# Edresson/VoiceSplit

Hardware: AMD Instinct MI355X
Metric: utterances/sec (3 s clips, B=64/GPU) fwd+bwd, channels-last bf16 activations / tape, bf16 MFMA, fp32 accumulate / statistics / master weights (higher is better)
Workload: dtype bf16 (conv activations and tape stored as bf16; bf16 MFMA operands in the convs, the LSTM / head contractions and the BPTT, f16 operands in the forward recurrence; fp32 accumulate, BatchNorm statistics, gate arithmetic / cell state, loss head, master weights)

## Files before the change

include/voicesplit_hip.h:

```cpp
#ifndef VOICESPLIT_HIP_H
#define VOICESPLIT_HIP_H

#include <stddef.h>
#include <stdint.h>

#ifdef __cplusplus
extern "C" {
#endif
#if defined(__GNUC__)
#pragma GCC visibility push(default)
#endif

#define VS_ABI_VERSION 10

#define VS_ACT_RELU 0
#define VS_ACT_MISH 1
#define VS_ACT_NONE 2
#define VS_ACT_SIGMOID 3

#define VS_MATH_FP32 0
#define VS_MATH_F16X3 1
#define VS_MATH_BF16 2

#define VS_BN_EVAL 0
#define VS_BN_TRAIN 1

typedef struct vs_dims {
  int B;
// ... 140 lines not shown
int vs_nhwc_bn_act_bwd(const void* da, const void* z, void* dz, long long npix, int act, int bn_mode,
                       const float* scale, const float* shift, const float* mean, const float* invstd,
                       float* dgamma, float* dbeta, float* dbias, double* stats, float* coef, void* stream);
int vs_nhwc_bn_act_bwd_first(const void* da, const void* z, const float* x, int B, int T, int F, int act, int bn_mode,
                             const float* scale, const float* shift, const float* mean, const float* invstd,
                             float* dgamma, float* dbeta, float* dbias, float* dw, double* stats, float* coef, double* acc, void* stream);
int vs_nhwc_conv_last_bwd_blocks(void);
int vs_nhwc_conv_last_bwd(const float* dz8, const float* w, const void* a7, void* din, float* partials, float* dw,
                          int B, int T, int F, void* stream);
int vs_nhwc_conv_dy(const void* dz, const void* packed, void* dy, const void* z, int act,
                    const float* bn_scale, const float* bn_shift, const float* bn_mean, const float* bn_invstd, double* bn_stats,
                    int B, int T, int F, int KT, int KF, int dil, void* stream);
int vs_nhwc_conv_last_bwd_dy(const float* dz8, const float* w, const void* a7, void* dy, float* partials, float* dw,
                             const void* z7, int act, const float* bn_scale, const float* bn_shift, const float* bn_mean,
                             const float* bn_invstd, double* bn_stats, int B, int T, int F, void* stream);
int vs_nhwc_bn_bwd_from_dy(const void* dy, const void* z, void* dz, long long npix, int bn_mode,
                           const float* scale, const float* mean, const float* invstd,
                           float* dgamma, float* dbeta, float* dbias, double* stats, float* coef, void* stream);
int vs_nhwc_bn_bwd_first_from_dy(const void* dy, const void* z, const float* x, int B, int T, int F, int bn_mode,
                                 const float* scale, const float* mean, const float* invstd,
                                 float* dgamma, float* dbeta, float* dbias, float* dw, double* stats, float* coef, double* acc, void* stream);
int vs_conv_last_fwd(const float* in, const float* w, const float* scale, const float* shift,
                     float* out, int B, int T, int F, int act, void* stream);
int vs_gemm_nt(const float* A, int lda, const float* W, int ldw, float* C, int ldc, int M, int N, int K,
               const float* bias1, const float* bias2, const float* rowbias, int ldrb, int group,
               int a_relu, int act, void* stream);
size_t vs_lstm_packed_floats(int H);
size_t vs_lstm_state_floats(int B, int H);
int vs_lstm_pack(const float* w_hh_fwd, const float* w_hh_bwd, float* packed, int H, void* stream);
int vs_bilstm_recurrent(const float* xg, const float* packed_whh, float* state, float* out,
// ... 149 lines not shown
```

voicesplit_amd/_lib.py:

```python
import ctypes
import os
from ctypes import POINTER, Structure, c_char_p, c_float, c_int, c_longlong, c_size_t, c_void_p

_HERE = os.path.dirname(os.path.abspath(__file__))
LIB_PATH = os.path.join(_HERE, "libvoicesplit_hip.so")

ACT_RELU, ACT_MISH, ACT_NONE, ACT_SIGMOID = 0, 1, 2, 3
BN_EVAL, BN_TRAIN = 0, 1
MATH_FP32, MATH_F16X3, MATH_BF16 = 0, 1, 2
PROF_SLOTS = 29
PROF_NAMES = ("cnn1", "cnn2", "cnn3", "cnn4", "cnn5", "cnn6", "cnn7", "cnn8", "lstm_gemm", "lstm_rec", "head",
              "fwd_bn", "bwd_head", "bwd_lstm_rec", "bwd_lstm_gemm", "bwd_bn",
              "wgrad_cnn2", "wgrad_cnn3", "wgrad_cnn4", "wgrad_cnn5", "wgrad_cnn6", "wgrad_cnn7",
              "dgrad_cnn2", "dgrad_cnn3", "dgrad_cnn4", "dgrad_cnn5", "dgrad_cnn6", "dgrad_cnn7", "bwd_edge")
ABI_VERSION = 10


class VsDims(Structure):
    _fields_ = [(n, c_int) for n in ("B", "T", "F", "E", "H", "FC1", "FC2", "math")]


class VsConvLayer(Structure):
    _fields_ = [(n, c_void_p) for n in ("weight", "bias", "bn_weight", "bn_bias",
                                        "bn_running_mean", "bn_running_var")]


class VsParams(Structure):
    _fields_ = [
        ("conv", VsConvLayer * 8),
        ("w_ih", c_void_p * 2), ("w_hh", c_void_p * 2), ("b_ih", c_void_p * 2), ("b_hh", c_void_p * 2),
# ... 83 lines not shown
    "vs_nhwc_first_stats": (c_int, [_P, _P, _P, ctypes.c_double, _P, _P]),
    "vs_nhwc_first_bwd_scratch_doubles": (c_int, []),
    "vs_nhwc_first_bwd": (c_int, [_P, _P, _P, _P, c_int, c_int, c_int, c_int, c_int, _P, _P, _P, _P, _P, _P, _P, _P, _P, _P]),
    "vs_bn_finalize": (c_int, [_P, c_int, ctypes.c_double, c_int, _P, _P, _P, _P, c_float, c_float, _P, _P, _P, _P, _P]),
    "vs_nhwc_bn_apply": (c_int, [_P, _P, c_longlong, c_int, _P, _P, _P]),
    "vs_nhwc_conv_last": (c_int, [_P, _P, _P, _P, _P, c_int, c_int, c_int, c_int, _P]),
    "vs_nhwc_conv_last_pre": (c_int, [_P, _P, _P, c_int, _P, _P, _P, _P, _P, c_int, c_int, c_int, _P]),
    "vs_nhwc_conv_wgrad_partial_floats": (c_size_t, [c_int, c_int]),
    "vs_nhwc_conv_wgrad": (c_int, [_P, _P, _P, _P, c_int, c_int, c_int, c_int, c_int, c_int, _P]),
    "vs_nhwc_bn_act_bwd": (c_int, [_P, _P, _P, c_longlong, c_int, c_int, _P, _P, _P, _P, _P, _P, _P, _P, _P, _P]),
    "vs_nhwc_bn_act_bwd_first": (c_int, [_P, _P, _P, c_int, c_int, c_int, c_int, c_int, _P, _P, _P, _P, _P, _P, _P, _P, _P, _P, _P, _P]),
    "vs_nhwc_conv_last_bwd_blocks": (c_int, []),
    "vs_nhwc_conv_last_bwd": (c_int, [_P, _P, _P, _P, _P, _P, c_int, c_int, c_int, _P]),
    "vs_nhwc_conv_dy": (c_int, [_P, _P, _P, _P, c_int, _P, _P, _P, _P, _P, c_int, c_int, c_int, c_int, c_int, c_int, _P]),
    "vs_nhwc_conv_last_bwd_dy": (c_int, [_P, _P, _P, _P, _P, _P, _P, c_int, _P, _P, _P, _P, _P, c_int, c_int, c_int, _P]),
    "vs_nhwc_bn_bwd_from_dy": (c_int, [_P, _P, _P, c_longlong, c_int, _P, _P, _P, _P, _P, _P, _P, _P, _P]),
    "vs_nhwc_bn_bwd_first_from_dy": (c_int, [_P, _P, _P, c_int, c_int, c_int, c_int, _P, _P, _P, _P, _P, _P, _P, _P, _P, _P, _P]),
    "vs_conv_last_fwd": (c_int, [_P, _P, _P, _P, _P, c_int, c_int, c_int, c_int, _P]),
    "vs_conv64_packed_f16_floats": (c_size_t, [c_int, c_int]),
    "vs_pow2_scale": (c_int, [_P, c_longlong, _P, _P, _P]),
    "vs_conv64_pack_f16": (c_int, [_P, _P, c_int, c_int, c_int, _P, _P, _P]),
    "vs_conv64_f16x3_fwd": (c_int, [_P, _P, _P, _P, _P, _P, _P, c_int, c_int, c_int, c_int, c_int, c_int, c_int, _P]),
    "vs_gemm_nt": (c_int, [_P, c_int, _P, c_int, _P, c_int, c_int, c_int, c_int, _P, _P, _P, c_int, c_int,
                           c_int, c_int, _P]),
    "vs_lstm_packed_floats": (c_size_t, [c_int]),
    "vs_lstm_state_floats": (c_size_t, [c_int, c_int]),
    "vs_lstm_pack": (c_int, [_P, _P, _P, c_int, _P]),
    "vs_bilstm_recurrent": (c_int, [_P, _P, _P, _P, c_int, c_int, c_int, _P]),
    "vs_lstm_pack_math": (c_int, [_P, _P, _P, c_int, c_int, _P]),
    "vs_bilstm_recurrent_math": (c_int, [_P, _P, _P, _P, _P, _P, c_int, c_int, c_int, c_int, _P]),
# ... 114 lines not shown
```

voicesplit_amd/csrc/capi.hip:

```cpp
#include <stdarg.h>
#include <stdlib.h>
#include <string.h>

#include "../../include/voicesplit_hip.h"
#include "vs_internal.h"

static thread_local char g_err[512] = "";

void vs_set_error(const char* fmt, ...) {
  va_list ap;
  va_start(ap, fmt);
  vsnprintf(g_err, sizeof(g_err), fmt, ap);
  va_end(ap);
}

int g_vs_options[VS_OPT_COUNT] = { 1,  1,  1,  1,  0,  0};
thread_local unsigned* g_vs_turn = nullptr;

namespace {
struct Prof {
  bool on = false;
  int max_calls = 0;
  int calls[VS_PROF_SLOTS] = {0};
  hipEvent_t* ev = nullptr;
// ... 450 lines not shown
  return vs_nhwc_bn_act_bwd_impl(da, z, dz, npix, act, bn_mode == VS_BN_TRAIN, scale, shift, mean, invstd, dgamma, dbeta, dbias,
                                 stats, coef, (hipStream_t)stream);
}

int vs_nhwc_bn_act_bwd_first(const void* da, const void* z, const float* x, int B, int T, int F, int act, int bn_mode,
                             const float* scale, const float* shift, const float* mean, const float* invstd,
                             float* dgamma, float* dbeta, float* dbias, float* dw, double* stats, float* coef, double* acc, void* stream) {
  return vs_nhwc_bn_act_bwd_first_impl(da, z, x, B, T, F, act, bn_mode == VS_BN_TRAIN, scale, shift, mean, invstd, dgamma, dbeta, dbias,
                                       dw, stats, coef, acc, (hipStream_t)stream);
}

int vs_nhwc_conv_last_bwd_blocks(void) { return VS_NHWC_LAST_BWD_BLOCKS; }

int vs_nhwc_conv_last_bwd(const float* dz8, const float* w, const void* a7, void* din, float* partials, float* dw,
                          int B, int T, int F, void* stream) {
  return vs_nhwc_conv_last_bwd_impl(dz8, w, a7, din, partials, dw, B, T, F, nullptr, VS_ACT_NONE, nullptr, nullptr, nullptr, nullptr, nullptr,
                                    (hipStream_t)stream);
}

int vs_nhwc_conv_dy(const void* dz, const void* packed, void* dy, const void* z, int act,
                    const float* bn_scale, const float* bn_shift, const float* bn_mean, const float* bn_invstd, double* bn_stats,
                    int B, int T, int F, int KT, int KF, int dil, void* stream) {
  VS_REQUIRE(dz != dy, "nhwc_conv_dy: in-place is not supported");
  return vs_nhwc_conv_dy_impl(dz, packed, dy, z, act, bn_scale, bn_shift, bn_mean, bn_invstd, bn_stats, B, T, F, KT, KF, dil, (hipStream_t)stream);
}

int vs_nhwc_conv_last_bwd_dy(const float* dz8, const float* w, const void* a7, void* dy, float* partials, float* dw,
                             const void* z7, int act, const float* bn_scale, const float* bn_shift, const float* bn_mean,
                             const float* bn_invstd, double* bn_stats, int B, int T, int F, void* stream) {
  VS_REQUIRE(z7, "nhwc_conv_last_bwd_dy: NULL z7");
  return vs_nhwc_conv_last_bwd_impl(dz8, w, a7, dy, partials, dw, B, T, F, z7, act, bn_scale, bn_shift, bn_mean, bn_invstd, bn_stats,
                                    (hipStream_t)stream);
}

int vs_nhwc_bn_bwd_from_dy(const void* dy, const void* z, void* dz, long long npix, int bn_mode,
                           const float* scale, const float* mean, const float* invstd,
                           float* dgamma, float* dbeta, float* dbias, double* stats, float* coef, void* stream) {
  return vs_nhwc_bn_bwd_from_dy_impl(dy, z, dz, npix, bn_mode == VS_BN_TRAIN, scale, mean, invstd, dgamma, dbeta, dbias, stats, coef,
                                     (hipStream_t)stream);
}

int vs_nhwc_bn_bwd_first_from_dy(const void* dy, const void* z, const float* x, int B, int T, int F, int bn_mode,
                                 const float* scale, const float* mean, const float* invstd,
                                 float* dgamma, float* dbeta, float* dbias, float* dw, double* stats, float* coef, double* acc, void* stream) {
  return vs_nhwc_bn_bwd_first_from_dy_impl(dy, z, x, B, T, F, bn_mode == VS_BN_TRAIN, scale, mean, invstd, dgamma, dbeta, dbias, dw,
                                           stats, coef, acc, (hipStream_t)stream);
}
// ... 393 lines not shown
```

voicesplit_amd/csrc/nhwc_edge.hip:

```cpp
#include "vs_internal.h"

namespace {

typedef unsigned u4v __attribute__((ext_vector_type(4)));
typedef unsigned u2v __attribute__((ext_vector_type(2)));

__device__ __forceinline__ float bf_lo(unsigned u) { return __uint_as_float(u << 16); }
__device__ __forceinline__ float bf_hi(unsigned u) { return __uint_as_float(u & 0xffff0000u); }

template <int NV>
__device__ __forceinline__ void fold_channel_sums(float (&v)[NV][8], double* __restrict__ stats, float* lds ,
                                                  unsigned* turn = nullptr) {
  const int lane = threadIdx.x & 63, wave = threadIdx.x >> 6;
#pragma unroll
  for (int q = 0; q < NV; ++q)
#pragma unroll
    for (int j = 0; j < 8; ++j) {
      float s = v[q][j];
      s += __shfl_xor(s, 8, 64);
      s += __shfl_xor(s, 16, 64);
      s += __shfl_xor(s, 32, 64);
      if (lane < 8) lds[(wave * NV + q) * 64 + lane * 8 + j] = s;
    }
  __syncthreads();
// ... 373 lines not shown
    const vs_f32x2 u = {__builtin_amdgcn_exp2f(e.x), __builtin_amdgcn_exp2f(e.y)};
    const vs_f32x2 n = u * (u + 2.0f);
    const vs_f32x2 dn = n + 2.0f;
    const vs_f32x2 r = {__builtin_amdgcn_rcpf(dn.x), __builtin_amdgcn_rcpf(dn.y)};
    a = y * (n * r);
    d = r * __builtin_elementwise_fma((yc * 4.0f) * r, __builtin_elementwise_fma(u, u, u), n);
  } else if (ACT == VS_ACT_RELU) {
    a = vs_f32x2{fmaxf(y.x, 0.0f), fmaxf(y.y, 0.0f)};
    d = vs_f32x2{y.x > 0.0f ? 1.0f : 0.0f, y.y > 0.0f ? 1.0f : 0.0f};
  } else {
    a = y;
    d = vs_f32x2{1.0f, 1.0f};
  }
}

template <int DYACT, bool RECOMP = false>
__global__ __launch_bounds__(256)
void nhwc_conv_last_bwd_kernel(const float* __restrict__ dz8, const float* __restrict__ w, const u4v* __restrict__ a7,
                               u4v* __restrict__ din, float* __restrict__ part, long long npix, int F, LastBwdBn bn) {
  __shared__ float red[4 * 8 * 64];
  const int piece = threadIdx.x & 7;
  vs_f32x2 wr[8][4], acc[8][4];
  vs_f32x2 sc[4], sh[4], mu[4], is[4], bacc[2][4];
#pragma unroll
  for (int co = 0; co < 8; ++co)
#pragma unroll
    for (int q = 0; q < 4; ++q) {
      wr[co][q] = vs_f32x2{w[co * 64 + piece * 8 + 2 * q], w[co * 64 + piece * 8 + 2 * q + 1]};
      acc[co][q] = vs_f32x2{0.f, 0.f};
    }
  if (DYACT >= 0) {
// ... 28 lines not shown
    if (fn >= F) { fn -= F; ++rown; }
    const long long pn = p + stride;
    if (pn < npix) fetch(pn, rown, fn, nxt);
    vs_f32x2 zf[4], dact[4];
    u4v av = cur.av;
    if (DYACT >= 0) {
#pragma unroll
      for (int q = 0; q < 4; ++q) {
        zf[q] = vs_f32x2{bf_lo(cur.zv[q]), bf_hi(cur.zv[q])};
        vs_f32x2 aq;
        nhwc_act_both2<(DYACT >= 0 ? DYACT : VS_ACT_NONE)>(__builtin_elementwise_fma(zf[q], sc[q], sh[q]), aq, dact[q]);
        if (RECOMP) av[q] = vs_pack_bf16(aq.x, aq.y);
      }
    }
    vs_f32x2 g[4];
#pragma unroll
    for (int q = 0; q < 4; ++q) g[q] = vs_f32x2{0.f, 0.f};
#pragma unroll
    for (int co = 0; co < 8; ++co) {
      const vs_f32x2 dd = {cur.d[co], cur.d[co]};
#pragma unroll
      for (int q = 0; q < 4; ++q) {
        g[q] = __builtin_elementwise_fma(wr[co][q], dd, g[q]);
        acc[co][q] = __builtin_elementwise_fma(dd, vs_f32x2{bf_lo(av[q]), bf_hi(av[q])}, acc[co][q]);
      }
    }
    if (DYACT >= 0) {
#pragma unroll
      for (int q = 0; q < 4; ++q) {
        g[q] *= dact[q];
        bacc[0][q] += g[q];
        bacc[1][q] = __builtin_elementwise_fma(g[q], (zf[q] - mu[q]) * is[q], bacc[1][q]);
      }
    }
    __builtin_nontemporal_store(u4v{vs_pack_bf16(g[0].x, g[0].y), vs_pack_bf16(g[1].x, g[1].y), vs_pack_bf16(g[2].x, g[2].y), vs_pack_bf16(g[3].x, g[3].y)},
                                din + p * 8 + piece);
    cur = nxt;
    f = fn;
    row = rown;
  }
  if (DYACT >= 0) {
    float b8[2][8];
#pragma unroll
    for (int q = 0; q < 4; ++q) {
      b8[0][2 * q] = bacc[0][q].x; b8[0][2 * q + 1] = bacc[0][q].y;
      b8[1][2 * q] = bacc[1][q].x; b8[1][2 * q + 1] = bacc[1][q].y;
    }
    fold_channel_sums<2>(b8, bn.stats, red, bn.turn);
    __syncthreads();
  }
  const int lane = threadIdx.x & 63, wave = threadIdx.x >> 6;
#pragma unroll
  for (int co = 0; co < 8; ++co)
#pragma unroll
    for (int j = 0; j < 8; ++j) {
      float s = (j & 1) ? acc[co][j >> 1].y : acc[co][j >> 1].x;
      s += __shfl_xor(s, 8, 64);
      s += __shfl_xor(s, 16, 64);
      s += __shfl_xor(s, 32, 64);
      if (lane < 8) red[(wave * 8 + co) * 64 + lane * 8 + j] = s;
    }
  __syncthreads();
  for (int i = threadIdx.x; i < 512; i += 256)
    part[(size_t)blockIdx.x * 512 + i] = red[i] + red[512 + i] + red[1024 + i] + red[1536 + i];
}

constexpr int kMomN = 7 + 28;

__global__ __launch_bounds__(256)
void nhwc_first_moments_kernel(const float* __restrict__ x, long long npix, int F, double* __restrict__ mom, unsigned* turn) {
  __shared__ float red[4][kMomN];
  float acc[kMomN];
#pragma unroll
  for (int i = 0; i < kMomN; ++i) acc[i] = 0.f;
  const long long stride = (long long)gridDim.x * 256;
  for (long long p = (long long)blockIdx.x * 256 + threadIdx.x; p < npix; p += stride) {
    const int f = (int)(p % F);
    const float* xr = x + (p - f);
    float xv[7];
// ... 404 lines not shown
  }
  if (int rc = vs_bn_bwd_finalize_impl(stats, VS_BN_STAT_SLOTS, (double)npix, train, 64, scale, mean, invstd, dgamma, dbeta, dbias, coef, stream)) return rc;
  VS_CHECK_HIP(hipMemsetAsync(acc, 0, sizeof(double) * 448, stream));
  const dim3 grid(stream_blocks(32, npix)), block(256);
  if (act == VS_ACT_MISH) hipLaunchKernelGGL(nhwc_bn_bwd_first_kernel<VS_ACT_MISH>, grid, block, 0, stream, g, zz, x, npix, F, scale, shift, coef, acc);
  else if (act == VS_ACT_RELU) hipLaunchKernelGGL(nhwc_bn_bwd_first_kernel<VS_ACT_RELU>, grid, block, 0, stream, g, zz, x, npix, F, scale, shift, coef, acc);
  else hipLaunchKernelGGL(nhwc_bn_bwd_first_kernel<VS_ACT_NONE>, grid, block, 0, stream, g, zz, x, npix, F, scale, shift, coef, acc);
  hipLaunchKernelGGL(nhwc_cvt_f64_f32_kernel, dim3(2), dim3(256), 0, stream, acc, dw, 448);
  VS_LAUNCH_CHECK();
  return 0;
}

int vs_nhwc_conv_last_bwd_impl(const float* dz8, const float* w, const void* a7, void* din, float* part, float* dw,
                               int B, int T, int F, const void* z7, int act, const float* bn_scale, const float* bn_shift,
                               const float* bn_mean, const float* bn_invstd, double* bn_stats, hipStream_t stream) {
  VS_REQUIRE(dz8 && w && din && part && dw, "nhwc conv_last_bwd: NULL argument");
  VS_REQUIRE(a7 || z7, "nhwc conv_last_bwd: a7 may only be NULL in the dy form (it is then recomputed from z7)");
  VS_REQUIRE(!z7 || (bn_scale && bn_shift && bn_mean && bn_invstd && bn_stats), "nhwc conv_last_bwd: the dy form needs the BatchNorm constants and statistics slots");
  const long long npix = (long long)B * T * F;
  long long nb = (npix + 31) / 32;
  if (nb > VS_NHWC_LAST_BWD_BLOCKS) nb = VS_NHWC_LAST_BWD_BLOCKS;
  const LastBwdBn bn{reinterpret_cast<const u4v*>(z7), bn_scale, bn_shift, bn_mean, bn_invstd, bn_stats, z7 ? g_vs_turn : nullptr};
  const dim3 grid((unsigned)nb), block(256);
  const u4v* a = reinterpret_cast<const u4v*>(a7);
  u4v* o = reinterpret_cast<u4v*>(din);
  if (!z7) hipLaunchKernelGGL(nhwc_conv_last_bwd_kernel<-1>, grid, block, 0, stream, dz8, w, a, o, part, npix, F, bn);
  else if (act == VS_ACT_MISH && !a7) hipLaunchKernelGGL((nhwc_conv_last_bwd_kernel<VS_ACT_MISH, true>), grid, block, 0, stream, dz8, w, a, o, part, npix, F, bn);
  else if (act == VS_ACT_RELU && !a7) hipLaunchKernelGGL((nhwc_conv_last_bwd_kernel<VS_ACT_RELU, true>), grid, block, 0, stream, dz8, w, a, o, part, npix, F, bn);
  else if (act == VS_ACT_MISH) hipLaunchKernelGGL(nhwc_conv_last_bwd_kernel<VS_ACT_MISH>, grid, block, 0, stream, dz8, w, a, o, part, npix, F, bn);
  else if (act == VS_ACT_RELU) hipLaunchKernelGGL(nhwc_conv_last_bwd_kernel<VS_ACT_RELU>, grid, block, 0, stream, dz8, w, a, o, part, npix, F, bn);
  else VS_REQUIRE(false, "nhwc conv_last_bwd: dy form for activation %d", act);
  VS_LAUNCH_CHECK();
  return vs_reduce_partials_impl(part, (int)nb, 512, dw, stream);
}

namespace {

typedef _Float16 h8v __attribute__((ext_vector_type(8)));
typedef _Float16 h2v __attribute__((ext_vector_type(2)));

__global__ void nhwc_first_plan_kernel(const unsigned* __restrict__ amax_in, int n_amax, const float* __restrict__ w, const float* __restrict__ scale,
                                       const float* __restrict__ shift, float* __restrict__ out_scale2, int nco, int taps) {
  const int c = threadIdx.x;
  unsigned mb = 0;
  for (int i = c; i < n_amax; i += 64) mb = amax_in[i] > mb ? amax_in[i] : mb;
#pragma unroll
  for (int o = 32; o > 0; o >>= 1) { const unsigned other = __shfl_xor(mb, o, 64); mb = other > mb ? other : mb; }
  float bound = 0.3125f;
// ... 265 lines not shown
```

voicesplit_amd/csrc/train.hip:

```cpp
#include <mutex>
#include <stdlib.h>
#include <string.h>

#include "../../include/voicesplit_hip.h"
#include "vs_internal.h"

int vs_check_dims_impl(const vs_dims* d);

namespace {

constexpr float kBnEps = 1e-5f;
constexpr float kBnMomentum = 0.1f;
struct Spec { int kt, kf, dil; };
constexpr Spec kMid[6] = {{7, 1, 1}, {5, 5, 1}, {5, 5, 2}, {5, 5, 4}, {5, 5, 8}, {5, 5, 16}};
constexpr int kSplitK = 16;

inline size_t align_up(size_t x) { return (x + 255) & ~size_t(255); }
template <typename T>
inline T* at(void* ws, size_t off) { return reinterpret_cast<T*>(static_cast<char*>(ws) + off); }
inline size_t max3(size_t a, size_t b, size_t c) { return a > b ? (a > c ? a : c) : (b > c ? b : c); }

int tape_layout(const vs_dims* d, vs_tape_layout* L) {
  if (int rc = vs_check_dims_impl(d)) return rc;
  memset(L, 0, sizeof(*L));
// ... 562 lines not shown
  auto bn_bwd = [&](int l, const float* da, const float* z, float* dz, int C, long long R, int Lrow) -> int {
    VsProfScope ps(VS_PROF_BWD_BN, stream);
    unsigned* amax = (f16 && l >= 1 && l <= 6) ? vs_amax_slot(cs + VS_SCALE_SLOT_FLOATS * (8 + l)) : nullptr;
    return vs_bn_act_bwd_impl(da, z, dz, C, R, Lrow, conv_act, train, scale + 64 * l, shift + 64 * l, mean + 64 * l,
                              invstd + 64 * l, g->conv[l].bn_weight, g->conv[l].bn_bias, g->conv[l].bias, stats, coef, amax, stream);
  };
  if (int rc = bn_bwd(7, dfeat, at<float>(tape, L.z8), dfeat, 8, (long long)M * 8, F)) return rc;
  if (d->math == VS_MATH_BF16) {
    const long long npix = (long long)B * T * F;
    void* gb[2] = {at<void>(tape, L.grad0), at<void>(tape, L.grad1)};
    int c = 0;
    constexpr int kStatsDoubles = 0;
    {
      VsProfScope ps(VS_PROF_BWD_EDGE, stream);
      VS_CHECK_HIP(hipMemsetAsync(stats, 0, sizeof(double) * VS_BN_STAT_SLOTS * 128, stream));
      if (int rc = vs_nhwc_conv_last_bwd_impl(dfeat, p->conv[7].weight, train ? nullptr : at<void>(tape, L.a[6]), gb[c], at<float>(tape, L.grad1),
                                              g->conv[7].weight, B, T, F, at<void>(tape, L.z[6]), conv_act, scale + 64 * 6, shift + 64 * 6,
                                              mean + 64 * 6, invstd + 64 * 6, stats, stream)) return rc;
    }
    {
      auto from_dy = [&](int l, void* gbuf, hipStream_t s, int beside) -> int {
        VsProfScope ps(VS_PROF_BWD_BN, s);
        return vs_nhwc_bn_bwd_from_dy_impl(gbuf, at<void>(tape, L.z[l]), gbuf, npix, train, scale + 64 * l, mean + 64 * l, invstd + 64 * l,
                                           g->conv[l].bn_weight, g->conv[l].bn_bias, g->conv[l].bias, stats, coef, s, kStatsDoubles, beside);
      };
      auto first_bwd = [&](void* gbuf, hipStream_t s) -> int {
        VsProfScope ps(VS_PROF_BWD_EDGE, s);
        return vs_nhwc_first_bwd_impl(gbuf, x, p->conv[0].weight, p->conv[0].bias, B, T, F, conv_act, train, scale, shift, mean, invstd,
                                      g->conv[0].bn_weight, g->conv[0].bn_bias, g->conv[0].bias, g->conv[0].weight,
                                      at<double>(tape, L.first_acc) + 64, s, at<double>(tape, L.first_acc),
                                      det ? at<double>(tape, L.det_turn) + VS_TURN_WORDS * 4 / 8 : nullptr);
      };
      if (int rc = from_dy(6, gb[c], stream, 0)) return rc;
      bool part_free = side == nullptr;
      for (int i = 5; i >= 0; --i) {
        const int l = i + 1;
        {
          VsProfScope ps(VS_PROF_BWD_DGRAD + i, stream);
          const void* pack_t = at<void>(tape, L.conv_packed_t[i]);
          if (l == 1) {
            if (int rc = vs_nhwc_conv_impl(gb[c], pack_t, ones, zeros, gb[c ^ 1], B, T, F, kMid[i].kt, kMid[i].kf, kMid[i].dil, VS_ACT_NONE,
                                           nullptr, stream)) return rc;
          } else {
            VS_CHECK_HIP(hipMemsetAsync(stats, 0, sizeof(double) * VS_BN_STAT_SLOTS * 128, stream));
            if (int rc = vs_nhwc_conv_dy_impl(gb[c], pack_t, gb[c ^ 1], at<void>(tape, L.z[l - 1]), conv_act, scale + 64 * (l - 1),
                                              shift + 64 * (l - 1), mean + 64 * (l - 1), invstd + 64 * (l - 1), stats,
                                              B, T, F, kMid[i].kt, kMid[i].kf, kMid[i].dil, stream)) return rc;
          }
// ... 209 lines not shown
```

voicesplit_amd/csrc/vs_internal.h:

```cpp
#pragma once
#include "vs_common.h"

struct VsProfScope {
  hipStream_t s; int idx;
  VsProfScope(int slot, hipStream_t s);
  ~VsProfScope();
};

extern int g_vs_options[VS_OPT_COUNT];
inline int vs_opt(int o) { return g_vs_options[o]; }
extern thread_local unsigned* g_vs_turn;
struct VsTurnScope {
  unsigned* prev;
  explicit VsTurnScope(unsigned* t) : prev(g_vs_turn) { g_vs_turn = t; }
  ~VsTurnScope() { g_vs_turn = prev; }
};
inline int vs_det_grid(int nb, int cus = 256) { return (g_vs_turn && nb > cus) ? cus : nb; }

int vs_conv64_pack_impl(const float* w, float* wp, int KT, int KF, int transpose_flip, hipStream_t);
int vs_conv64_fwd_impl(const float* in, const float* wp, const float* scale, const float* shift, float* out,
                       int B, int T, int F, int KT, int KF, int dil, int act, hipStream_t);
int vs_pow2_scale_impl(const float* x, long long n, unsigned* amax_scratch, float* scale2, hipStream_t);
int vs_scale_from_absmax_impl(const unsigned* amax, int n, float* scale2, hipStream_t);
int vs_absmax_accum_impl(const float* x, long long n, unsigned* amax, hipStream_t);
// ... 83 lines not shown
                           void* rows_bf16 = nullptr ,
                           int Kp = 0);
int vs_nhwc_bn_act_bwd_impl(const void* da, const void* z, void* dz, long long npix, int act, int train,
                            const float* scale, const float* shift, const float* mean, const float* invstd,
                            float* dgamma, float* dbeta, float* dbias, double* stats, float* coef, hipStream_t, int beside_wgrad = 0);
int vs_nhwc_bn_act_bwd_first_impl(const void* da, const void* z, const float* x, int B, int T, int F, int act, int train,
                                  const float* scale, const float* shift, const float* mean, const float* invstd,
                                  float* dgamma, float* dbeta, float* dbias, float* dw, double* stats, float* coef, double* acc, hipStream_t);
#define VS_NHWC_LAST_BWD_BLOCKS 1024
int vs_nhwc_conv_last_bwd_impl(const float* dz8, const float* w, const void* a7, void* din, float* part, float* dw,
                               int B, int T, int F, const void* z7, int act, const float* bn_scale, const float* bn_shift,
                               const float* bn_mean, const float* bn_invstd, double* bn_stats, hipStream_t stream);
int vs_nhwc_conv_dy_impl(const void* dz, const void* packed, void* dy, const void* z, int act,
                         const float* bn_scale, const float* bn_shift, const float* bn_mean, const float* bn_invstd, double* bn_stats,
                         int B, int T, int F, int KT, int KF, int dil, hipStream_t stream);
int vs_nhwc_bn_bwd_from_dy_impl(const void* dy, const void* z, void* dz, long long npix, int train,
                                const float* scale, const float* mean, const float* invstd,
                                float* dgamma, float* dbeta, float* dbias, double* stats, float* coef, hipStream_t stream, int rezero_doubles = 0,
                                int beside_wgrad = 0 );
int vs_nhwc_bn_bwd_first_from_dy_impl(const void* dy, const void* z, const float* x, int B, int T, int F, int train,
                                      const float* scale, const float* mean, const float* invstd,
                                      float* dgamma, float* dbeta, float* dbias, float* dw, double* stats, float* coef, double* acc,
                                      hipStream_t stream);
int vs_bn_bwd_finalize_impl(double* stats, int slots, double count, int train, int C, const float* scale, const float* mean,
                            const float* invstd, float* dgamma, float* dbeta, float* dbias, float* coef, hipStream_t,
                            int rezero_doubles = 0 );
int vs_bn_finalize_impl(double* stats, int slots, double count, int C, const float* gamma, const float* beta,
                        float* running_mean, float* running_var, float eps, float momentum,
                        float* scale, float* shift, float* mean_out, float* invstd_out, hipStream_t, int rezero_doubles = 0);
int vs_bn_fold_impl(const float*, const float*, const float*, const float*, const float*, float, int, float*, float*, hipStream_t);
// ... 73 lines not shown
```

voicesplit_amd/ops.py:

```python
import ctypes
import os
from typing import Dict, Optional, Sequence

import torch

from . import _lib
from ._lib import (ACT_MISH, ACT_NONE, ACT_RELU, ACT_SIGMOID, BN_EVAL, BN_TRAIN, VsDims, VsParams,
                   VsWsLayout, check)

ACT_CODES = {"relu": ACT_RELU, "mish": ACT_MISH, "none": ACT_NONE, "sigmoid": ACT_SIGMOID}

CONV_INDEX = ((1, 2), (5, 6), (9, 10), (13, 14), (17, 18), (21, 22), (25, 26), (28, 29))


def _dev_check(t: torch.Tensor, name: str, dtype=torch.float32):
    if not isinstance(t, torch.Tensor):
        raise TypeError(f"{name}: expected a tensor")
    if not t.is_cuda:
        raise _lib.VoiceSplitHipError(
            f"{name} is on {t.device}: this path only runs on an MI355X (HIP) device; there is no CPU fallback")
    if t.dtype != dtype:
        raise TypeError(f"{name}: expected {dtype}, got {t.dtype}")
    if not t.is_contiguous():
        raise ValueError(f"{name}: must be contiguous")
# ... 791 lines not shown
    lib = _lib.load()
    _dev_check(dz8, "dz8")
    if a7 is not None:
        _dev_check(a7, "a7", torch.bfloat16)
    _dev_check(z7, "z7", torch.bfloat16)
    B, T, F, _ = z7.shape
    dy = torch.empty_like(z7)
    part = torch.empty(lib.vs_nhwc_conv_last_bwd_blocks() * 512, dtype=torch.float32, device=z7.device)
    dw = torch.empty(8, 64, dtype=torch.float32, device=z7.device)
    stats = torch.zeros(64, 64, 2, dtype=torch.float64, device=z7.device)
    check(lib.vs_nhwc_conv_last_bwd_dy(_p(dz8), _p(w), _p(a7), _p(dy), _p(part), _p(dw), _p(z7), ACT_CODES[act], _p(bn_scale), _p(bn_shift),
                                       _p(bn_mean), _p(bn_invstd), _p(stats), B, T, F, _stream()), "vs_nhwc_conv_last_bwd_dy")
    return dy, dw, stats


def nhwc_bn_bwd_from_dy(dy, z, stats, training: bool, scale, mean, invstd):
    lib = _lib.load()
    _dev_check(dy, "dy", torch.bfloat16)
    _dev_check(z, "z", torch.bfloat16)
    dev = z.device
    dz = torch.empty_like(dy)
    dg, db, dbias = (torch.empty(64, dtype=torch.float32, device=dev) for _ in range(3))
    coef = torch.empty(192, dtype=torch.float32, device=dev)
    check(lib.vs_nhwc_bn_bwd_from_dy(_p(dy), _p(z), _p(dz), z.numel() // 64, BN_TRAIN if training else BN_EVAL, _p(scale), _p(mean),
                                     _p(invstd), _p(dg), _p(db), _p(dbias), _p(stats), _p(coef), _stream()), "vs_nhwc_bn_bwd_from_dy")
    return dz, dg, db, dbias


def nhwc_bn_bwd_first_from_dy(dy, z, x, stats, training: bool, scale, mean, invstd):
    lib = _lib.load()
# ... 62 lines not shown
```

Measured before the change: 1459.

## Split last-conv backward into stats sweep and fused apply sweep, skipping dy round-trip

```diff
diff --git a/include/voicesplit_hip.h b/include/voicesplit_hip.h
--- a/include/voicesplit_hip.h
+++ b/include/voicesplit_hip.h
@@ -11,7 +11,7 @@
 #pragma GCC visibility push(default)
 #endif
 
-#define VS_ABI_VERSION 10
+#define VS_ABI_VERSION 11
 
 #define VS_ACT_RELU 0
 #define VS_ACT_MISH 1
@@ -182,6 +182,11 @@
 int vs_nhwc_conv_last_bwd_dy(const float* dz8, const float* w, const void* a7, void* dy, float* partials, float* dw,
                              const void* z7, int act, const float* bn_scale, const float* bn_shift, const float* bn_mean,
                              const float* bn_invstd, double* bn_stats, int B, int T, int F, void* stream);
+int vs_nhwc_last_bwd_sums(const float* dz8, const float* w, const void* z7, int act, const float* bn_scale, const float* bn_shift,
+                          const float* bn_mean, const float* bn_invstd, double* bn_stats, float* partials, int B, int T, int F, void* stream);
+int vs_nhwc_last_bwd_apply(const float* dz8, const float* w, const void* z7, int act, int bn_mode, const float* bn_scale, const float* bn_shift,
+                           const float* bn_mean, const float* bn_invstd, double* bn_stats, float* dgamma, float* dbeta, float* dbias, float* coef,
+                           const float* partials, float* dw, void* dz7, int B, int T, int F, void* stream);
 int vs_nhwc_bn_bwd_from_dy(const void* dy, const void* z, void* dz, long long npix, int bn_mode,
                            const float* scale, const float* mean, const float* invstd,
                            float* dgamma, float* dbeta, float* dbias, double* stats, float* coef, void* stream);
diff --git a/voicesplit_amd/_lib.py b/voicesplit_amd/_lib.py
--- a/voicesplit_amd/_lib.py
+++ b/voicesplit_amd/_lib.py
@@ -13,7 +13,7 @@
               "fwd_bn", "bwd_head", "bwd_lstm_rec", "bwd_lstm_gemm", "bwd_bn",
               "wgrad_cnn2", "wgrad_cnn3", "wgrad_cnn4", "wgrad_cnn5", "wgrad_cnn6", "wgrad_cnn7",
               "dgrad_cnn2", "dgrad_cnn3", "dgrad_cnn4", "dgrad_cnn5", "dgrad_cnn6", "dgrad_cnn7", "bwd_edge")
-ABI_VERSION = 10
+ABI_VERSION = 11
 
 
 class VsDims(Structure):
@@ -127,6 +127,8 @@
     "vs_nhwc_conv_last_bwd": (c_int, [_P, _P, _P, _P, _P, _P, c_int, c_int, c_int, _P]),
     "vs_nhwc_conv_dy": (c_int, [_P, _P, _P, _P, c_int, _P, _P, _P, _P, _P, c_int, c_int, c_int, c_int, c_int, c_int, _P]),
     "vs_nhwc_conv_last_bwd_dy": (c_int, [_P, _P, _P, _P, _P, _P, _P, c_int, _P, _P, _P, _P, _P, c_int, c_int, c_int, _P]),
+    "vs_nhwc_last_bwd_sums": (c_int, [_P, _P, _P, c_int, _P, _P, _P, _P, _P, _P, c_int, c_int, c_int, _P]),
+    "vs_nhwc_last_bwd_apply": (c_int, [_P, _P, _P, c_int, c_int, _P, _P, _P, _P, _P, _P, _P, _P, _P, _P, _P, _P, c_int, c_int, c_int, _P]),
     "vs_nhwc_bn_bwd_from_dy": (c_int, [_P, _P, _P, c_longlong, c_int, _P, _P, _P, _P, _P, _P, _P, _P, _P]),
     "vs_nhwc_bn_bwd_first_from_dy": (c_int, [_P, _P, _P, c_int, c_int, c_int, c_int, _P, _P, _P, _P, _P, _P, _P, _P, _P, _P, _P]),
     "vs_conv_last_fwd": (c_int, [_P, _P, _P, _P, _P, c_int, c_int, c_int, c_int, _P]),
diff --git a/voicesplit_amd/csrc/capi.hip b/voicesplit_amd/csrc/capi.hip
--- a/voicesplit_amd/csrc/capi.hip
+++ b/voicesplit_amd/csrc/capi.hip
@@ -488,6 +488,7 @@
 
 int vs_nhwc_conv_last_bwd(const float* dz8, const float* w, const void* a7, void* din, float* partials, float* dw,
                           int B, int T, int F, void* stream) {
+  VS_REQUIRE(din && dw, "nhwc_conv_last_bwd: NULL argument");
   return vs_nhwc_conv_last_bwd_impl(dz8, w, a7, din, partials, dw, B, T, F, nullptr, VS_ACT_NONE, nullptr, nullptr, nullptr, nullptr, nullptr,
                                     (hipStream_t)stream);
 }
@@ -503,8 +504,27 @@
                              const void* z7, int act, const float* bn_scale, const float* bn_shift, const float* bn_mean,
                              const float* bn_invstd, double* bn_stats, int B, int T, int F, void* stream) {
   VS_REQUIRE(z7, "nhwc_conv_last_bwd_dy: NULL z7");
+  VS_REQUIRE(dy && dw, "nhwc_conv_last_bwd_dy: NULL argument");
   return vs_nhwc_conv_last_bwd_impl(dz8, w, a7, dy, partials, dw, B, T, F, z7, act, bn_scale, bn_shift, bn_mean, bn_invstd, bn_stats,
                                     (hipStream_t)stream);
+}
+
+int vs_nhwc_last_bwd_sums(const float* dz8, const float* w, const void* z7, int act, const float* bn_scale, const float* bn_shift,
+                          const float* bn_mean, const float* bn_invstd, double* bn_stats, float* partials, int B, int T, int F, void* stream) {
+  VS_REQUIRE(dz8 && w && z7 && partials, "nhwc_last_bwd_sums: NULL argument");
+  return vs_nhwc_last_bwd_sums_impl(dz8, w, z7, act, bn_scale, bn_shift, bn_mean, bn_invstd, bn_stats, partials, B, T, F, (hipStream_t)stream);
+}
+
+int vs_nhwc_last_bwd_apply(const float* dz8, const float* w, const void* z7, int act, int bn_mode, const float* bn_scale, const float* bn_shift,
+                           const float* bn_mean, const float* bn_invstd, double* bn_stats, float* dgamma, float* dbeta, float* dbias, float* coef,
+                           const float* partials, float* dw, void* dz7, int B, int T, int F, void* stream) {
+  VS_REQUIRE(dz8 && w && z7 && bn_scale && bn_shift && bn_mean && bn_invstd && bn_stats && dgamma && dbeta && dbias && coef && partials && dw && dz7,
+             "nhwc_last_bwd_apply: NULL argument");
+  VS_REQUIRE(B > 0 && T > 0 && F > 0, "nhwc_last_bwd_apply: bad shape");
+  hipStream_t s = (hipStream_t)stream;
+  if (int rc = vs_bn_bwd_finalize_impl(bn_stats, VS_BN_STAT_SLOTS, (double)B * T * F, bn_mode == VS_BN_TRAIN, 64, bn_scale, bn_mean, bn_invstd,
+                                       dgamma, dbeta, dbias, coef, s)) return rc;
+  return vs_nhwc_last_bwd_apply_impl(dz8, w, z7, act, bn_scale, bn_shift, coef, partials, dw, dz7, B, T, F, s);
 }
 
 int vs_nhwc_bn_bwd_from_dy(const void* dy, const void* z, void* dz, long long npix, int bn_mode,
diff --git a/voicesplit_amd/csrc/nhwc_edge.hip b/voicesplit_amd/csrc/nhwc_edge.hip
--- a/voicesplit_amd/csrc/nhwc_edge.hip
+++ b/voicesplit_amd/csrc/nhwc_edge.hip
@@ -411,7 +411,18 @@
   }
 }
 
-template <int DYACT, bool RECOMP = false>
+__device__ __forceinline__ void last_bwd_da(const float (&d)[8], const vs_f32x2 (&wr)[8][4], vs_f32x2 (&g)[4]) {
+#pragma unroll
+  for (int q = 0; q < 4; ++q) g[q] = vs_f32x2{0.f, 0.f};
+#pragma unroll
+  for (int co = 0; co < 8; ++co) {
+    const vs_f32x2 dd = {d[co], d[co]};
+#pragma unroll
+    for (int q = 0; q < 4; ++q) g[q] = __builtin_elementwise_fma(wr[co][q], dd, g[q]);
+  }
+}
+
+template <int DYACT, bool RECOMP = false, bool STORE = true>
 __global__ __launch_bounds__(256)
 void nhwc_conv_last_bwd_kernel(const float* __restrict__ dz8, const float* __restrict__ w, const u4v* __restrict__ a7,
                                u4v* __restrict__ din, float* __restrict__ part, long long npix, int F, LastBwdBn bn) {
@@ -470,16 +481,12 @@
       }
     }
     vs_f32x2 g[4];
-#pragma unroll
-    for (int q = 0; q < 4; ++q) g[q] = vs_f32x2{0.f, 0.f};
+    last_bwd_da(cur.d, wr, g);
 #pragma unroll
     for (int co = 0; co < 8; ++co) {
       const vs_f32x2 dd = {cur.d[co], cur.d[co]};
 #pragma unroll
-      for (int q = 0; q < 4; ++q) {
-        g[q] = __builtin_elementwise_fma(wr[co][q], dd, g[q]);
-        acc[co][q] = __builtin_elementwise_fma(dd, vs_f32x2{bf_lo(av[q]), bf_hi(av[q])}, acc[co][q]);
-      }
+      for (int q = 0; q < 4; ++q) acc[co][q] = __builtin_elementwise_fma(dd, vs_f32x2{bf_lo(av[q]), bf_hi(av[q])}, acc[co][q]);
     }
     if (DYACT >= 0) {
 #pragma unroll
@@ -489,8 +496,9 @@
         bacc[1][q] = __builtin_elementwise_fma(g[q], (zf[q] - mu[q]) * is[q], bacc[1][q]);
       }
     }
-    __builtin_nontemporal_store(u4v{vs_pack_bf16(g[0].x, g[0].y), vs_pack_bf16(g[1].x, g[1].y), vs_pack_bf16(g[2].x, g[2].y), vs_pack_bf16(g[3].x, g[3].y)},
-                                din + p * 8 + piece);
+    if (STORE)
+      __builtin_nontemporal_store(u4v{vs_pack_bf16(g[0].x, g[0].y), vs_pack_bf16(g[1].x, g[1].y), vs_pack_bf16(g[2].x, g[2].y), vs_pack_bf16(g[3].x, g[3].y)},
+                                  din + p * 8 + piece);
     cur = nxt;
     f = fn;
     row = rown;
@@ -519,6 +527,109 @@
   __syncthreads();
   for (int i = threadIdx.x; i < 512; i += 256)
     part[(size_t)blockIdx.x * 512 + i] = red[i] + red[512 + i] + red[1024 + i] + red[1536 + i];
+}
+
+constexpr int kApplySteps = 8;
+
+template <int ACT>
+__global__ __launch_bounds__(256)
+void nhwc_last_bwd_apply_kernel(const float* __restrict__ dz8, const float* __restrict__ w, const u2v* __restrict__ z7,
+                                const float* __restrict__ scale, const float* __restrict__ shift, const float* __restrict__ coef,
+                                u2v* __restrict__ dz, long long npix, int F, const float* __restrict__ part, int nparts, float* __restrict__ dw) {
+  typedef float f32x4 __attribute__((ext_vector_type(4)));
+  if (dw && blockIdx.x < 4 && threadIdx.x < 128) {
+    const int c = blockIdx.x * 128 + threadIdx.x;
+    float s = 0.f;
+    int gq = 0;
+    for (; gq + 16 <= nparts; gq += 16) {
+      float v[16];
+#pragma unroll
+      for (int u = 0; u < 16; ++u) v[u] = part[(size_t)(gq + u) * 512 + c];
+#pragma unroll
+      for (int u = 0; u < 16; ++u) s += v[u];
+    }
+    for (; gq < nparts; ++gq) s += part[(size_t)gq * 512 + c];
+    dw[c] = s;
+  }
+  const int lane = threadIdx.x & 63, wave = threadIdx.x >> 6;
+  const int j = lane & 15, gk = lane >> 4;
+  float bw[4][2];
+#pragma unroll
+  for (int m = 0; m < 4; ++m)
+#pragma unroll
+    for (int s = 0; s < 2; ++s) bw[m][s] = w[(4 * s + gk) * 64 + 4 * j + m];
+  vs_f32x2 sc[2], sh[2], cA[2], cB[2], cC[2];
+#pragma unroll
+  for (int q = 0; q < 2; ++q) {
+    const int c = 4 * j + 2 * q;
+    sc[q] = vs_f32x2{scale[c], scale[c + 1]}; sh[q] = vs_f32x2{shift[c], shift[c + 1]};
+    cA[q] = vs_f32x2{coef[c], coef[c + 1]}; cB[q] = vs_f32x2{coef[64 + c], coef[64 + c + 1]}; cC[q] = vs_f32x2{coef[128 + c], coef[128 + c + 1]};
+  }
+  const long long wbase = ((long long)blockIdx.x * 4 + wave) * (16 * kApplySteps);
+  if (wbase >= npix) return;
+  const long long wend = wbase + 16 * kApplySteps < npix ? wbase + 16 * kApplySteps : npix;
+  const int sr = 16 % F;
+  const int sq = 16 / F;
+  long long pa = wbase + j;
+  long long row = pa / F;
+  int f = (int)(pa - row * F);
+  struct In { float a[2]; u2v z[4]; };
+  auto fetch = [&](long long pb, long long pq, long long rq, int fq, In& in) {
+    if (pq < npix) {
+      const float* d = dz8 + rq * 8 * F + fq;
+      in.a[0] = d[(size_t)gk * F];
+      in.a[1] = d[(size_t)(4 + gk) * F];
+    } else {
+      in.a[0] = in.a[1] = 0.f;
+    }
+#pragma unroll
+    for (int r = 0; r < 4; ++r) {
+      const long long pz = pb + 4 * gk + r;
+      in.z[r] = pz < npix ? __builtin_nontemporal_load(z7 + pz * 16 + j) : u2v{0u, 0u};
+    }
+  };
+  In cur, nxt;
+  long long pb = wbase;
+  fetch(pb, pa, row, f, cur);
+  for (; pb < wend; pb += 16) {
+    int fn = f + sr;
+    long long rown = row + sq;
+    if (fn >= F) { fn -= F; ++rown; }
+    const long long pan = pa + 16;
+    if (pb + 16 < wend) fetch(pb + 16, pan, rown, fn, nxt);
+    f32x4 d[4];
+#pragma unroll
+    for (int m = 0; m < 4; ++m) {
+      d[m] = __builtin_amdgcn_mfma_f32_16x16x4f32(cur.a[0], bw[m][0], f32x4{0.f, 0.f, 0.f, 0.f}, 0, 0, 0);
+      d[m] = __builtin_amdgcn_mfma_f32_16x16x4f32(cur.a[1], bw[m][1], d[m], 0, 0, 0);
+    }
+#pragma unroll
+    for (int r = 0; r < 4; ++r) {
+      u2v o;
+#pragma unroll
+      for (int q = 0; q < 2; ++q) {
+        const vs_f32x2 zf = {bf_lo(cur.z[r][q]), bf_hi(cur.z[r][q])};
+        vs_f32x2 aq, dact;
+        nhwc_act_both2<ACT>(__builtin_elementwise_fma(zf, sc[q], sh[q]), aq, dact);
+        vs_f32x2 g = vs_f32x2{d[2 * q][r], d[2 * q + 1][r]};
+        g *= dact;
+        const unsigned dy = vs_pack_bf16(g.x, g.y);
+        o[q] = vs_pack_bf16(fmaf(cA[q].x, bf_lo(dy), fmaf(cB[q].x, zf.x, cC[q].x)), fmaf(cA[q].y, bf_hi(dy), fmaf(cB[q].y, zf.y, cC[q].y)));
+      }
+      const long long pz = pb + 4 * gk + r;
+      if (pz < npix) __builtin_nontemporal_store(o, dz + pz * 16 + j);
+    }
+    cur = nxt;
+    pa = pan;
+    f = fn;
+    row = rown;
+  }
+}
+
+int last_bwd_blocks(long long npix) {
+  long long nb = (npix + 31) / 32;
+  if (nb > VS_NHWC_LAST_BWD_BLOCKS) nb = VS_NHWC_LAST_BWD_BLOCKS;
+  return (int)nb;
 }
 
 constexpr int kMomN = 7 + 28;
@@ -953,24 +1064,62 @@
 int vs_nhwc_conv_last_bwd_impl(const float* dz8, const float* w, const void* a7, void* din, float* part, float* dw,
                                int B, int T, int F, const void* z7, int act, const float* bn_scale, const float* bn_shift,
                                const float* bn_mean, const float* bn_invstd, double* bn_stats, hipStream_t stream) {
-  VS_REQUIRE(dz8 && w && din && part && dw, "nhwc conv_last_bwd: NULL argument");
+  VS_REQUIRE(dz8 && w && part, "nhwc conv_last_bwd: NULL argument");
+  VS_REQUIRE(din || z7, "nhwc conv_last_bwd: din may only be NULL in the dy form (sweep 1 of the edge sweeps)");
+  VS_REQUIRE(din || !dw, "nhwc conv_last_bwd: sweep 1 leaves the dW8 partials to sweep 2");
   VS_REQUIRE(a7 || z7, "nhwc conv_last_bwd: a7 may only be NULL in the dy form (it is then recomputed from z7)");
   VS_REQUIRE(!z7 || (bn_scale && bn_shift && bn_mean && bn_invstd && bn_stats), "nhwc conv_last_bwd: the dy form needs the BatchNorm constants and statistics slots");
+  VS_REQUIRE(B > 0 && T > 0 && F > 0, "nhwc conv_last_bwd: bad shape");
   const long long npix = (long long)B * T * F;
-  long long nb = (npix + 31) / 32;
-  if (nb > VS_NHWC_LAST_BWD_BLOCKS) nb = VS_NHWC_LAST_BWD_BLOCKS;
+  const long long nb = last_bwd_blocks(npix);
   const LastBwdBn bn{reinterpret_cast<const u4v*>(z7), bn_scale, bn_shift, bn_mean, bn_invstd, bn_stats, z7 ? g_vs_turn : nullptr};
   const dim3 grid((unsigned)nb), block(256);
   const u4v* a = reinterpret_cast<const u4v*>(a7);
   u4v* o = reinterpret_cast<u4v*>(din);
-  if (!z7) hipLaunchKernelGGL(nhwc_conv_last_bwd_kernel<-1>, grid, block, 0, stream, dz8, w, a, o, part, npix, F, bn);
+  if (!din) {
+    VS_REQUIRE(!a7, "nhwc conv_last_bwd: sweep 1 recomputes a7");
+    if (act == VS_ACT_MISH) hipLaunchKernelGGL((nhwc_conv_last_bwd_kernel<VS_ACT_MISH, true, false>), grid, block, 0, stream, dz8, w, a, o, part, npix, F, bn);
+    else if (act == VS_ACT_RELU) hipLaunchKernelGGL((nhwc_conv_last_bwd_kernel<VS_ACT_RELU, true, false>), grid, block, 0, stream, dz8, w, a, o, part, npix, F, bn);
+    else VS_REQUIRE(false, "nhwc conv_last_bwd: sweep 1 for activation %d", act);
+  } else if (!z7) hipLaunchKernelGGL(nhwc_conv_last_bwd_kernel<-1>, grid, block, 0, stream, dz8, w, a, o, part, npix, F, bn);
   else if (act == VS_ACT_MISH && !a7) hipLaunchKernelGGL((nhwc_conv_last_bwd_kernel<VS_ACT_MISH, true>), grid, block, 0, stream, dz8, w, a, o, part, npix, F, bn);
   else if (act == VS_ACT_RELU && !a7) hipLaunchKernelGGL((nhwc_conv_last_bwd_kernel<VS_ACT_RELU, true>), grid, block, 0, stream, dz8, w, a, o, part, npix, F, bn);
   else if (act == VS_ACT_MISH) hipLaunchKernelGGL(nhwc_conv_last_bwd_kernel<VS_ACT_MISH>, grid, block, 0, stream, dz8, w, a, o, part, npix, F, bn);
   else if (act == VS_ACT_RELU) hipLaunchKernelGGL(nhwc_conv_last_bwd_kernel<VS_ACT_RELU>, grid, block, 0, stream, dz8, w, a, o, part, npix, F, bn);
   else VS_REQUIRE(false, "nhwc conv_last_bwd: dy form for activation %d", act);
   VS_LAUNCH_CHECK();
-  return vs_reduce_partials_impl(part, (int)nb, 512, dw, stream);
+  return dw ? vs_reduce_partials_impl(part, (int)nb, 512, dw, stream) : 0;
+}
+
+int vs_nhwc_last_bwd_sums_impl(const float* dz8, const float* w, const void* z7, int act, const float* bn_scale, const float* bn_shift,
+                               const float* bn_mean, const float* bn_invstd, double* bn_stats, float* part, int B, int T, int F,
+                               hipStream_t stream) {
+  VS_REQUIRE(z7, "nhwc last_bwd_sums: NULL z7");
+  VS_REQUIRE(act == VS_ACT_MISH || act == VS_ACT_RELU, "nhwc last_bwd_sums: activation %d", act);
+  return vs_nhwc_conv_last_bwd_impl(dz8, w, nullptr, nullptr, part, nullptr, B, T, F, z7, act, bn_scale, bn_shift, bn_mean, bn_invstd,
+                                    bn_stats, stream);
+}
+
+int vs_nhwc_last_bwd_apply_impl(const float* dz8, const float* w, const void* z7, int act, const float* bn_scale, const float* bn_shift,
+                                const float* coef, const float* part, float* dw, void* dz7, int B, int T, int F, hipStream_t stream) {
+  VS_REQUIRE(dz8 && w && z7 && bn_scale && bn_shift && coef && part && dw && dz7, "nhwc last_bwd_apply: NULL argument");
+  VS_REQUIRE(dz7 != z7, "nhwc last_bwd_apply: dz7 may not alias z7");
+  VS_REQUIRE(B > 0 && T > 0 && F > 0, "nhwc last_bwd_apply: bad shape");
+  const long long npix = (long long)B * T * F;
+  long long nb = (npix + 64 * kApplySteps - 1) / (64 * kApplySteps);
+  if (nb < 4) nb = 4;
+  VS_REQUIRE(nb <= 0x7fffffffLL, "nhwc last_bwd_apply: %lld pixels", npix);
+  const dim3 grid((unsigned)nb), block(256);
+  const u2v* z = reinterpret_cast<const u2v*>(z7);
+  u2v* o = reinterpret_cast<u2v*>(dz7);
+  const int nparts = last_bwd_blocks(npix);
+  if (act == VS_ACT_MISH)
+    hipLaunchKernelGGL(nhwc_last_bwd_apply_kernel<VS_ACT_MISH>, grid, block, 0, stream, dz8, w, z, bn_scale, bn_shift, coef, o, npix, F, part, nparts, dw);
+  else if (act == VS_ACT_RELU)
+    hipLaunchKernelGGL(nhwc_last_bwd_apply_kernel<VS_ACT_RELU>, grid, block, 0, stream, dz8, w, z, bn_scale, bn_shift, coef, o, npix, F, part, nparts, dw);
+  else VS_REQUIRE(false, "nhwc last_bwd_apply: activation %d", act);
+  VS_LAUNCH_CHECK();
+  return 0;
 }
 
 namespace {
diff --git a/voicesplit_amd/csrc/train.hip b/voicesplit_amd/csrc/train.hip
--- a/voicesplit_amd/csrc/train.hip
+++ b/voicesplit_amd/csrc/train.hip
@@ -600,9 +600,14 @@
     {
       VsProfScope ps(VS_PROF_BWD_EDGE, stream);
       VS_CHECK_HIP(hipMemsetAsync(stats, 0, sizeof(double) * VS_BN_STAT_SLOTS * 128, stream));
-      if (int rc = vs_nhwc_conv_last_bwd_impl(dfeat, p->conv[7].weight, train ? nullptr : at<void>(tape, L.a[6]), gb[c], at<float>(tape, L.grad1),
-                                              g->conv[7].weight, B, T, F, at<void>(tape, L.z[6]), conv_act, scale + 64 * 6, shift + 64 * 6,
-                                              mean + 64 * 6, invstd + 64 * 6, stats, stream)) return rc;
+      if (train) {
+        if (int rc = vs_nhwc_last_bwd_sums_impl(dfeat, p->conv[7].weight, at<void>(tape, L.z[6]), conv_act, scale + 64 * 6, shift + 64 * 6,
+                                                mean + 64 * 6, invstd + 64 * 6, stats, at<float>(tape, L.grad1), B, T, F, stream)) return rc;
+      } else {
+        if (int rc = vs_nhwc_conv_last_bwd_impl(dfeat, p->conv[7].weight, at<void>(tape, L.a[6]), gb[c], at<float>(tape, L.grad1),
+                                                g->conv[7].weight, B, T, F, at<void>(tape, L.z[6]), conv_act, scale + 64 * 6, shift + 64 * 6,
+                                                mean + 64 * 6, invstd + 64 * 6, stats, stream)) return rc;
+      }
     }
     {
       auto from_dy = [&](int l, void* gbuf, hipStream_t s, int beside) -> int {
@@ -617,7 +622,15 @@
                                       at<double>(tape, L.first_acc) + 64, s, at<double>(tape, L.first_acc),
                                       det ? at<double>(tape, L.det_turn) + VS_TURN_WORDS * 4 / 8 : nullptr);
       };
-      if (int rc = from_dy(6, gb[c], stream, 0)) return rc;
+      if (train) {
+        VsProfScope ps(VS_PROF_BWD_BN, stream);
+        if (int rc = vs_bn_bwd_finalize_impl(stats, VS_BN_STAT_SLOTS, (double)npix, train, 64, scale + 64 * 6, mean + 64 * 6, invstd + 64 * 6,
+                                             g->conv[6].bn_weight, g->conv[6].bn_bias, g->conv[6].bias, coef, stream, kStatsDoubles)) return rc;
+        if (int rc = vs_nhwc_last_bwd_apply_impl(dfeat, p->conv[7].weight, at<void>(tape, L.z[6]), conv_act, scale + 64 * 6, shift + 64 * 6,
+                                                 coef, at<float>(tape, L.grad1), g->conv[7].weight, gb[c], B, T, F, stream)) return rc;
+      } else {
+        if (int rc = from_dy(6, gb[c], stream, 0)) return rc;
+      }
       bool part_free = side == nullptr;
       for (int i = 5; i >= 0; --i) {
         const int l = i + 1;
diff --git a/voicesplit_amd/csrc/vs_internal.h b/voicesplit_amd/csrc/vs_internal.h
--- a/voicesplit_amd/csrc/vs_internal.h
+++ b/voicesplit_amd/csrc/vs_internal.h
@@ -121,6 +121,11 @@
 int vs_nhwc_conv_dy_impl(const void* dz, const void* packed, void* dy, const void* z, int act,
                          const float* bn_scale, const float* bn_shift, const float* bn_mean, const float* bn_invstd, double* bn_stats,
                          int B, int T, int F, int KT, int KF, int dil, hipStream_t stream);
+int vs_nhwc_last_bwd_sums_impl(const float* dz8, const float* w, const void* z7, int act, const float* bn_scale, const float* bn_shift,
+                               const float* bn_mean, const float* bn_invstd, double* bn_stats, float* part, int B, int T, int F,
+                               hipStream_t stream);
+int vs_nhwc_last_bwd_apply_impl(const float* dz8, const float* w, const void* z7, int act, const float* bn_scale, const float* bn_shift,
+                                const float* coef, const float* part, float* dw, void* dz7, int B, int T, int F, hipStream_t stream);
 int vs_nhwc_bn_bwd_from_dy_impl(const void* dy, const void* z, void* dz, long long npix, int train,
                                 const float* scale, const float* mean, const float* invstd,
                                 float* dgamma, float* dbeta, float* dbias, double* stats, float* coef, hipStream_t stream, int rezero_doubles = 0,
diff --git a/voicesplit_amd/ops.py b/voicesplit_amd/ops.py
--- a/voicesplit_amd/ops.py
+++ b/voicesplit_amd/ops.py
@@ -829,6 +829,34 @@
     return dy, dw, stats
 
 
+def nhwc_last_bwd_sums(dz8, w, z7, act: str, bn_scale, bn_shift, bn_mean, bn_invstd):
+    lib = _lib.load()
+    _dev_check(dz8, "dz8")
+    _dev_check(z7, "z7", torch.bfloat16)
+    B, T, F, _ = z7.shape
+    part = torch.empty(lib.vs_nhwc_conv_last_bwd_blocks() * 512, dtype=torch.float32, device=z7.device)
+    stats = torch.zeros(64, 64, 2, dtype=torch.float64, device=z7.device)
+    check(lib.vs_nhwc_last_bwd_sums(_p(dz8), _p(w), _p(z7), ACT_CODES[act], _p(bn_scale), _p(bn_shift), _p(bn_mean), _p(bn_invstd),
+                                    _p(stats), _p(part), B, T, F, _stream()), "vs_nhwc_last_bwd_sums")
+    return stats, part
+
+
+def nhwc_last_bwd_apply(dz8, w, z7, act: str, training: bool, bn_scale, bn_shift, bn_mean, bn_invstd, stats, part):
+    lib = _lib.load()
+    _dev_check(dz8, "dz8")
+    _dev_check(z7, "z7", torch.bfloat16)
+    B, T, F, _ = z7.shape
+    dev = z7.device
+    dz = torch.empty_like(z7)
+    dw = torch.empty(8, 64, dtype=torch.float32, device=dev)
+    dg, db, dbias = (torch.empty(64, dtype=torch.float32, device=dev) for _ in range(3))
+    coef = torch.empty(192, dtype=torch.float32, device=dev)
+    check(lib.vs_nhwc_last_bwd_apply(_p(dz8), _p(w), _p(z7), ACT_CODES[act], BN_TRAIN if training else BN_EVAL, _p(bn_scale), _p(bn_shift),
+                                     _p(bn_mean), _p(bn_invstd), _p(stats), _p(dg), _p(db), _p(dbias), _p(coef), _p(part), _p(dw), _p(dz),
+                                     B, T, F, _stream()), "vs_nhwc_last_bwd_apply")
+    return dz, dw, dg, db, dbias
+
+
 def nhwc_bn_bwd_from_dy(dy, z, stats, training: bool, scale, mean, invstd):
     lib = _lib.load()
     _dev_check(dy, "dy", torch.bfloat16)
```

New measurement: 1460 (median of 5 runs). Within noise of the previous version (+0.0%).
